# adityabalu/DiffNet

Hardware: NVIDIA B200
Metric: FEM loss+grad throughput (higher is better)
Workload: dtype f32

## Files before the change

diffnet_b200/csrc/dn_api.cu:

```cuda
#include <cstdarg>
#include <cstdio>
#include <cstdlib>
#include <cstring>

#include "dn_common.cuh"
#include "fem2d.cuh"
#include "fem2d_tma.cuh"
#include "fem3d.cuh"
#include "gp_eval.cuh"

namespace dn {
int debug_plan3t(const dn_geom* g, int nfields, int has_nu, int64_t* out);
cudaError_t launch_peer_put(float* dst_peer, const float* src, size_t n, int* remote_flag, int* local_counter,
                            unsigned int* ticket, cudaStream_t s);
cudaError_t launch_peer_wait(float* halo, const float* staged, size_t n, const int* flag, int* expect,
                             long long max_spins, int* status, cudaStream_t s);
cudaError_t launch_peer_loss_sum(const double* slots, int world, const int* step, long long max_spins, int* status,
                                 float* out, cudaStream_t s);
cudaError_t launch_peer_allreduce(const float* partial, float* out, double* slots, double* const* peer_slots,
                                  int rank, int world, int* counter, long long max_spins, int* status,
                                  cudaStream_t s);
}

namespace dn {
// ... 40 lines not shown
  }
  if (!g_dev[dev].ok) return fail(DN_EARCH, "device %d is not sm_100", dev);
  if (sms) *sms = g_dev[dev].sms;
  return DN_OK;
}

static int gauss_rule(int n, double* x, double* w) {
  switch (n) {
    case 2: x[0] = -0.5773502691896258; x[1] = 0.5773502691896258; w[0] = w[1] = 1.0; return 0;
    case 3: x[0] = -0.774596669; x[1] = 0.0; x[2] = 0.774596669;
            w[0] = 5.0 / 9.0; w[1] = 8.0 / 9.0; w[2] = 5.0 / 9.0; return 0;
    case 4: x[0] = -0.861136; x[1] = -0.339981; x[2] = 0.339981; x[3] = 0.861136;
            w[0] = 0.347855; w[1] = 0.652145; w[2] = 0.652145; w[3] = 0.347855; return 0;
  }
  return -1;
}

static Field to_field(const dn_field* f) {
  Field o{nullptr, 0, 0, 0};
  if (f && f->ptr) { o.p = f->ptr; o.sb = f->stride_b; o.sz = f->stride_z; o.sy = f->stride_y; }
  return o;
}

static bool aligned4(const Field& f, bool use_z) {
  if (!f.p) return true;
  return ((uintptr_t)f.p % 16 == 0) && (f.sb % 4 == 0) && (f.sy % 4 == 0) && (!use_z || f.sz % 4 == 0);
}

struct Common {
  Field u, nu, f, fgp, numask;
  Mask mk[DN_MAX_MASKS];
  int nmasks, MK;
  Consts k;
  Rule rule;
  bool vec4;
};

static int prepare(const dn_field* u, const dn_field* nu, const dn_field* f, const dn_field* fgp,
                   const dn_mask* masks, int nmasks, const dn_field* nu_zero_mask,
                   const dn_geom* g, double c_k, double c_f, double S, int nsd, Common* c, int flags = 0) {
  if (!g) return fail(DN_EINVAL, "geom is NULL");
  if (g->nsd != nsd) return fail(DN_EINVAL, "geom.nsd=%d but the %d-D entry point was called", g->nsd, nsd);
  if (g->batch < 1 || g->nx < 2 || g->ny < 2 || (nsd == 3 && g->nz < 2))
    return fail(DN_EINVAL, "need batch >= 1 and >= 2 nodes per direction (B=%d nx=%d ny=%d nz=%d)",
                g->batch, g->nx, g->ny, g->nz);
  if (!(g->hx > 0) || !(g->hy > 0) || (nsd == 3 && !(g->hz > 0)))
    return fail(DN_EINVAL, "element sizes must be positive");
  if (!u || !u->ptr) return fail(DN_EINVAL, "u is NULL");
  if (f && f->ptr && fgp && fgp->ptr) return fail(DN_EINVAL, "give f or fgp, not both");
  if ((flags & DN_F_LOAD_VECTOR) && !(f && f->ptr)) return fail(DN_EINVAL, "DN_F_LOAD_VECTOR needs the load vector in f");
  if (nmasks < 0 || nmasks > DN_MAX_MASKS)
    return fail(DN_EINVAL, "nmasks=%d (max %d)", nmasks, DN_MAX_MASKS);
  if (nmasks > 0 && !masks) return fail(DN_EINVAL, "masks is NULL");
  double gx[4], gw[4];
  if (gauss_rule(g->ngp_1d, gx, gw)) return fail(DN_EINVAL, "ngp_1d=%d (2..4)", g->ngp_1d);

  c->u = to_field(u); c->nu = to_field(nu); c->f = to_field(f); c->fgp = to_field(fgp);
  c->numask = to_field(nu_zero_mask);
  if (c->numask.p && !c->nu.p) return fail(DN_EINVAL, "nu_zero_mask needs nu");
  c->nmasks = nmasks;
  int nvf = 0;
  for (int i = 0; i < DN_MAX_MASKS; ++i) c->mk[i] = Mask{{nullptr, 0, 0, 0}, {nullptr, 0, 0, 0}, 0.f};
  for (int i = 0; i < nmasks; ++i) {
    if (!masks[i].mask.ptr) return fail(DN_EINVAL, "masks[%d].mask is NULL", i);
    c->mk[i].m = to_field(&masks[i].mask);
    c->mk[i].vf = to_field(&masks[i].value_field);
    c->mk[i].v = masks[i].value;
    nvf += c->mk[i].vf.p ? 1 : 0;
  }
  if (nvf > 0 && nmasks != 1)
    return fail(DN_EINVAL, "a Dirichlet value_field is supported only as the single mask");
  c->MK = nvf ? 4 : nmasks;

  double W1 = 0, m2 = 0;
  for (int i = 0; i < g->ngp_1d; ++i) { W1 += gw[i]; m2 += gw[i] * gx[i] * gx[i]; }
  const double t = m2 / W1;
  const double Wn = (nsd == 2) ? W1 * W1 : W1 * W1 * W1;
  const double nrm = (nsd == 2) ? 64.0 : 512.0;
  c->k.kx = (float)(S * c_k * Wn * (2.0 / g->hx) * (2.0 / g->hx) / nrm);
  c->k.ky = (float)(S * c_k * Wn * (2.0 / g->hy) * (2.0 / g->hy) / nrm);
  c->k.kz = (nsd == 3) ? (float)(S * c_k * Wn * (2.0 / g->hz) * (2.0 / g->hz) / nrm) : 0.f;
  c->k.kf = (float)(S * c_f * Wn / ((nsd == 2) ? 16.0 : 64.0));
  c->k.t = (float)t;
  c->k.kb = (float)(S * c_f);
  c->k.lv = (flags & DN_F_LOAD_VECTOR) ? 1 : 0;
  c->rule.n = g->ngp_1d;
  for (int i = 0; i < 4; ++i) {
    c->rule.x[i] = i < g->ngp_1d ? (float)gx[i] : 0.f;
    c->rule.w[i] = i < g->ngp_1d ? (float)gw[i] : 0.f;
  }
  c->rule.fscale = (float)(((nsd == 2) ? 4.0 : 8.0) / Wn);

  bool v4 = (g->nx % 4 == 0);
  const bool z = (nsd == 3);
  v4 = v4 && aligned4(c->u, z) && aligned4(c->nu, z) && aligned4(c->f, z) && aligned4(c->numask, z);
  for (int i = 0; i < nmasks; ++i) v4 = v4 && aligned4(c->mk[i].m, z) && aligned4(c->mk[i].vf, z);
  if (env_int("DN_FORCE_SCALAR", 0)) v4 = false;
  c->vec4 = v4;
  return DN_OK;
}

struct Plan2D { int V, R, nchunks, ntx, nitems, wpc, grid; };

static Plan2D plan2d(const dn_geom* g, bool vec4, int sms) {
  Plan2D pl;
  pl.V = vec4 ? 4 : 1;
  pl.ntx = (g->nx + 32 * pl.V - 1) / (32 * pl.V);
  const long long target = (long long)sms * env_int("DN_WARPS_PER_SM_2D", 16);
  long long per_row_items = (long long)g->batch * pl.ntx;
  long long want = (target + per_row_items - 1) / per_row_items;
  if (want < 1) want = 1;
  int R = (int)((g->ny + want - 1) / want);
  const int Rmin = env_int("DN_RMIN_2D", 8);
  if (R < Rmin) R = Rmin;
  if (R > g->ny) R = g->ny;
// ... 77 lines not shown
  if (!c.vec4 || c.fgp.p || ((uintptr_t)grad % 16 != 0)) return DN_OK;
  const int NU = c.nu.p ? 1 : 0, F = c.f.p ? (c.k.lv ? 2 : 1) : 0, NMK = c.numask.p ? 1 : 0;
  if (g->nx % 4 != 0 || g->nx / 4 > DN_T2_MAXT) return DN_OK;
  int MKx = c.MK;
  if (!mask_input) {
    if (c.MK == 0) MKx = 0;
    else if (c.MK >= 1 && c.MK <= 3 && !F && !NMK) MKx = c.MK + 4;
    else return DN_OK;
  }
  launch2t_fn fn = get_launch2t(MKx, NU, F, NMK);
  occ2t_fn occ = get_occ2t(MKx, NU, F, NMK);
  if (!fn || !occ) return DN_OK;
  P2T p;
  memset(&p, 0, sizeof(p));
  int nf = 0;
  p.fld[nf++] = c.u;
  if (NU) p.fld[nf++] = c.nu;
  if (F) p.fld[nf++] = c.f;
  if (NMK) p.fld[nf++] = c.numask;
  for (int i = 0; i < c.nmasks; ++i) { p.fld[nf++] = c.mk[i].m; p.mval[i] = c.mk[i].v; }
  if (c.MK == 4) p.fld[nf++] = c.mk[0].vf;
  for (int i = 0; i < nf; ++i)
    if (p.fld[i].sy != g->nx) return DN_OK;
  Plan2T pl = plan2t(g, nf, sms, occ);
  if (!pl.ok) { cudaGetLastError(); return DN_OK; }
  if (pl.grid > 0x7fffffffLL) return DN_OK;
  if (!workspace || wsb < ws_bytes_for_grid(pl.grid))
    return fail(DN_EWORKSPACE, "workspace too small: %zu < %zu", wsb, ws_bytes_for_grid(pl.grid));
  if ((uintptr_t)workspace % 16) return fail(DN_EWORKSPACE, "workspace must be 16-byte aligned");
  p.nf = nf;
  p.B = g->batch; p.nx = g->nx; p.ny = g->ny;
  p.R = pl.R; p.nchunks = pl.nchunks; p.S = pl.S;
  p.bal_q = pl.bal_q; p.bal_rem = pl.bal_rem;
  const float kx = c.k.kx, ky = c.k.ky, kf = c.k.kf, t = c.k.t;
  p.k2.kx = make_float2(kx, kx); p.k2.ky = make_float2(ky, ky); p.k2.t = make_float2(t, t);
  p.k2.kxt = make_float2(kx * t, kx * t); p.k2.kyt = make_float2(ky * t, ky * t);
  p.k2.nkf = make_float2(-kf, -kf); p.k2.nkft = make_float2(-kf * t, -kf * t);
  p.k2.nkftt = make_float2(-kf * t * t, -kf * t * t);
  p.k2.c0x_const = make_float2(4.f * kx, 4.f * kx); p.k2.c0y_const = make_float2(4.f * ky, 4.f * ky);
  p.k2.nkb = make_float2(-c.k.kb, -c.k.kb);
  p.grad = grad;
  p.red.counter = (unsigned int*)workspace;
  p.red.partials = (double*)((char*)workspace + 64);
  p.red.loss_out = loss_out; p.red.loss_f32 = loss_f32;
  p.mode = mode;
  *handled = true;
  return check_cuda(fn(p, dim3((unsigned)pl.grid), dim3(pl.threads), pl.smem, (cudaStream_t)stream),
                    "fem2d_tma launch");
}

static int run2d(const Common& c, const dn_geom* g, float* grad, float* grad_nu, int mode,
                 int mask_input, void* workspace, size_t wsb, double* loss_out, float* loss_f32,
                 void* stream, int sms) {
  if (!grad_nu) {
    bool handled = false;
    int rc = run2t(c, g, grad, mode, mask_input, workspace, wsb, loss_out, loss_f32, stream, sms, &handled);
    if (rc != DN_OK || handled) return rc;
  }
  if (c.k.lv)
    return fail(DN_ENOSTREAM, "DN_F_LOAD_VECTOR: the streaming 2-D kernel cannot take this launch (nx %% 4, nx <= %d, "
                "16-byte aligned dense rows, no grad_nu); pass f_gp instead", 4 * DN_T2_MAXT);
  bool vec4 = c.vec4 && ((uintptr_t)grad % 16 == 0) && ((uintptr_t)grad_nu % 16 == 0);
  Plan2D pl = plan2d(g, vec4, sms);
  if (!workspace || wsb < ws_bytes_for_grid(pl.grid))
    return fail(DN_EWORKSPACE, "workspace too small: %zu < %zu", wsb, ws_bytes_for_grid(pl.grid));
  if ((uintptr_t)workspace % 16) return fail(DN_EWORKSPACE, "workspace must be 16-byte aligned");
  P2D p;
  memset(&p, 0, sizeof(p));
  p.u = c.u; p.nu = c.nu; p.f = c.f; p.fgp = c.fgp; p.numask = c.numask;
  for (int i = 0; i < DN_MAX_MASKS; ++i) p.mk[i] = c.mk[i];
  p.B = g->batch; p.nx = g->nx; p.ny = g->ny;
// ... 396 lines not shown
```

diffnet_b200/csrc/fem2d_tma.cuh:

```cuda
#pragma once
#include <cstdlib>
#include <cstring>
#include <type_traits>

#include "dn_common.cuh"

namespace dn {

#define DN_T2_MAXF 8
#define DN_T2_MAXT 512

struct K2 {
  float2 kx, ky, kxt, kyt, t, nkf, nkft, nkftt, c0x_const, c0y_const;
  float2 nkb;
};

struct P2T {
  Field fld[DN_T2_MAXF];
  float mval[DN_MAX_MASKS];
  int nf;
  int B, nx, ny;
  int R, nchunks, S;
  int bal_q, bal_rem;
  K2 k2;
  float* grad;
  Reduce red;
  int mode;
};

__device__ __forceinline__ uint32_t smem_u32(const void* p) {
  return (uint32_t)__cvta_generic_to_shared(p);
}
__device__ __forceinline__ void mbar_init(uint64_t* bar, uint32_t count) {
  asm volatile("mbarrier.init.shared::cta.b64 [%0], %1;" ::"r"(smem_u32(bar)), "r"(count));
}
__device__ __forceinline__ void fence_mbar_init() {
  asm volatile("fence.mbarrier_init.release.cluster;" ::: "memory");
}
__device__ __forceinline__ void mbar_arrive_expect_tx(uint64_t* bar, uint32_t bytes) {
  asm volatile("mbarrier.arrive.expect_tx.shared::cta.b64 _, [%0], %1;" ::"r"(smem_u32(bar)),
               "r"(bytes)
               : "memory");
}
__device__ __forceinline__ void bulk_g2s(void* dst, const void* src, uint32_t bytes, uint64_t* bar) {
  asm volatile(
      "cp.async.bulk.shared::cluster.global.mbarrier::complete_tx::bytes [%0], [%1], %2, [%3];" ::"r"(
          smem_u32(dst)),
// ... 13 lines not shown
      "DN_DONE:\n"
      "}" ::"r"(smem_u32(bar)),
      "r"(parity)
      : "memory");
}

__device__ __forceinline__ void sts_if(bool pred, float* p, float v) {
  asm volatile("{\n.reg .pred P;\nsetp.ne.u32 P, %0, 0;\n@P st.shared.f32 [%1], %2;\n}" ::"r"((unsigned)pred), "r"(smem_u32(p)), "f"(v)
               : "memory");
}

__device__ __forceinline__ float2 f2(float a, float b) { return make_float2(a, b); }
__device__ __forceinline__ float2 f2(float a) { return make_float2(a, a); }
__device__ __forceinline__ float2 add2(float2 a, float2 b) { return __fadd2_rn(a, b); }
__device__ __forceinline__ float2 sub2(float2 a, float2 b) {
  return __fadd2_rn(a, make_float2(-b.x, -b.y));
}
__device__ __forceinline__ float2 mul2(float2 a, float2 b) { return __fmul2_rn(a, b); }
__device__ __forceinline__ float2 fma2(float2 a, float2 b, float2 c) { return __ffma2_rn(a, b, c); }

struct RowSD {
  float2 s01, s23, d01, d23;
};
__device__ __forceinline__ RowSD row_sd(const float (&v)[5]) {
  RowSD o;
  o.s01 = f2(v[0] + v[1], v[1] + v[2]);
  o.s23 = f2(v[2] + v[3], v[3] + v[4]);
  o.d01 = f2(v[1] - v[0], v[2] - v[1]);
  o.d23 = f2(v[3] - v[2], v[4] - v[3]);
  return o;
}


template <bool HAS_NU, bool HAS_F>
__device__ __forceinline__ float2 elem_pair(const K2& k, float2 st, float2 dt, float2 sb, float2 db,
                                            float2 nst, float2 ndt, float2 nsb, float2 ndb,
                                            float2 fst, float2 fdt, float2 fsb, float2 fdb,
                                            float2 vw, float2& ga, float2& gb, float2& gc,
                                            float2& gd) {
  const float2 Ae = sub2(sb, st), Ax = add2(dt, db), Axe = sub2(db, dt);
  float2 c0x, c0y, qx, qe, qxe;
  const float2 tAxe = mul2(k.t, Axe);
  if constexpr (HAS_NU) {
    const float2 C0 = add2(nst, nsb), Ce = sub2(nsb, nst), Cx = add2(ndt, ndb);
    c0x = mul2(k.kx, C0);
    c0y = mul2(k.ky, C0);
    const float2 c1x = mul2(k.kxt, Ce), c1y = mul2(k.kyt, Cx);
    qx = fma2(c0x, Ax, mul2(c1x, Axe));
    qe = fma2(c0y, Ae, mul2(c1y, Axe));
    qxe = fma2(add2(c0x, c0y), tAxe, fma2(c1x, Ax, mul2(c1y, Ae)));
  } else {
    c0x = mul2(k.c0x_const, vw);
    c0y = mul2(k.c0y_const, vw);
    qx = mul2(c0x, Ax);
    qe = mul2(c0y, Ae);
    qxe = mul2(add2(c0x, c0y), tAxe);
  }
  float2 E, g0, gx, ge, gxe;
  if constexpr (HAS_F) {
    const float2 A0 = add2(st, sb);
    const float2 nb0 = mul2(k.nkf, add2(fst, fsb));
    const float2 tx = fma2(k.nkft, add2(fdt, fdb), qx);
    const float2 te = fma2(k.nkft, sub2(fsb, fst), qe);
    const float2 txe = fma2(k.nkftt, sub2(fdb, fdt), qxe);
    E = fma2(A0, nb0, fma2(Ax, tx, fma2(Ae, te, mul2(Axe, txe))));
    g0 = nb0; gx = add2(qx, tx); ge = add2(qe, te); gxe = add2(qxe, txe);
    const float2 m0 = sub2(g0, ge), m1 = add2(g0, ge), n0 = sub2(gx, gxe), n1 = add2(gx, gxe);
    ga = sub2(m0, n0); gb = add2(m0, n0); gc = sub2(m1, n1); gd = add2(m1, n1);
  } else {
    E = fma2(Ax, qx, fma2(Ae, qe, mul2(Axe, qxe)));
    gx = add2(qx, qx); ge = add2(qe, qe); gxe = add2(qxe, qxe);
    const float2 n0 = sub2(gx, gxe), n1 = add2(gx, gxe);
    ga = sub2(f2(-ge.x, -ge.y), n0); gb = sub2(n0, ge); gc = sub2(ge, n1); gd = add2(ge, n1);
  }
  return E;
}

struct Row2T {
  RowSD u, n, f;
  float2 keep01, keep23;
  float2 lb01, lb23;
  float lE;
};
struct Acc2T {
  float2 a01, a23;
  float a4;
};

template <int NM, bool VF, bool HAS_NU, int FK, bool NUMASK, bool MI = true>
struct Fem2T {
  static constexpr bool HAS_F = (FK == 1), LV = (FK == 2);
  static constexpr int NF = 1 + (HAS_NU ? 1 : 0) + (FK ? 1 : 0) + (NUMASK ? 1 : 0) + NM + (VF ? 1 : 0);
  static constexpr int F_U = 0, F_NU = 1, F_F = F_NU + (HAS_NU ? 1 : 0), F_NM = F_F + (FK ? 1 : 0),
                       F_M = F_NM + (NUMASK ? 1 : 0), F_VF = F_M + NM;

  static __device__ __forceinline__ void load_row(const P2T& p, const float* __restrict__ sp, int fstride,
                                                  bool has_right, Row2T& o) {
    float v[NF][5];
#pragma unroll
    for (int f = 0; f < NF; ++f) {
      const float* q = sp + f * fstride;
      const float4 t = *reinterpret_cast<const float4*>(q);
      const float h = q[4];
      v[f][0] = t.x; v[f][1] = t.y; v[f][2] = t.z; v[f][3] = t.w; v[f][4] = has_right ? h : 0.f;
    }
    float ub[5], nb[5], fb[5], kp[4];
#pragma unroll
    for (int e = 0; e < 5; ++e) {
      float u = v[F_U][e];
      bool fx = false;
#pragma unroll
      for (int m = 0; m < NM; ++m) {
        const bool hit = v[F_M + m][e] > 0.5f;
        if constexpr (MI) u = hit ? (VF ? v[F_VF][e] : p.mval[m]) : u;
        fx = fx || hit;
      }
      ub[e] = u;
      if (e < 4) kp[e] = fx ? 0.f : 1.f;
      if constexpr (HAS_NU) {
        float n = v[F_NU][e];
        if constexpr (NUMASK) n = (v[F_NM][e] > 0.5f) ? 0.f : n;
        nb[e] = n;
      }
      if constexpr (HAS_F || LV) fb[e] = v[F_F][e];
    }
    o.keep01 = f2(kp[0], kp[1]);
    o.keep23 = f2(kp[2], kp[3]);
    if constexpr (LV) {
      o.lb01 = mul2(p.k2.nkb, f2(fb[0], fb[1]));
      o.lb23 = mul2(p.k2.nkb, f2(fb[2], fb[3]));
      const float2 le = fma2(o.lb01, f2(ub[0], ub[1]), mul2(o.lb23, f2(ub[2], ub[3])));
      o.lE = le.x + le.y;
    }
    o.u = row_sd(ub);
    if constexpr (HAS_NU) {
      o.n = row_sd(nb);
      if (!has_right) { o.n.s23.y = 0.f; o.n.d23.y = 0.f; }
    }
    if constexpr (HAS_F) {
      o.f = row_sd(fb);
      if (!has_right) { o.f.s23.y = 0.f; o.f.d23.y = 0.f; }
    }
  }

  static __device__ __forceinline__ float elem_row(const K2& k, const Row2T& top, const Row2T& bot,
                                                   float2 vw01, float2 vw23, Acc2T& At, Acc2T& Ab) {
    float2 ga, gb, gc, gd;
    const float2 E0 = elem_pair<HAS_NU, HAS_F>(k, top.u.s01, top.u.d01, bot.u.s01, bot.u.d01,
                                              top.n.s01, top.n.d01, bot.n.s01, bot.n.d01,
                                              top.f.s01, top.f.d01, bot.f.s01, bot.f.d01, vw01,
                                              ga, gb, gc, gd);
    At.a01 = add2(At.a01, ga);
    At.a01.y += gb.x; At.a23.x += gb.y;
    Ab.a01 = gc; Ab.a01.y += gd.x;
    const float carry = gd.y;
    const float2 E1 = elem_pair<HAS_NU, HAS_F>(k, top.u.s23, top.u.d23, bot.u.s23, bot.u.d23,
                                              top.n.s23, top.n.d23, bot.n.s23, bot.n.d23,
                                              top.f.s23, top.f.d23, bot.f.s23, bot.f.d23, vw23,
                                              ga, gb, gc, gd);
    At.a23 = add2(At.a23, ga);
    At.a23.y += gb.x; At.a4 += gb.y;
    Ab.a23 = gc; Ab.a23.x += carry; Ab.a23.y += gd.x;
    Ab.a4 = gd.y;
    const float2 Es = add2(E0, E1);
    return Es.x + Es.y;
  }
};

__device__ __forceinline__ unsigned int draw_start_ticket(const Reduce& r) { return atomicAdd(r.counter, 1u); }

__device__ __forceinline__ long long ld_relaxed_b64(const void* p) {
  long long v;
  asm volatile("ld.relaxed.gpu.global.b64 %0, [%1];" : "=l"(v) : "l"(p) : "memory");
  return v;
}

template <int NB = 40>
__device__ __forceinline__ void finish_loss_w0(const Reduce& r, double cta_value, unsigned int start_ticket) {
  if (threadIdx.x >= 32) return;
  const int lane = threadIdx.x;
  unsigned fin = 0u;
  if (lane == 0) {
    long long bits = __double_as_longlong(cta_value);
    if ((bits << 1) == 0) bits = (long long)0x8000000000000000ull;
    __stcg(reinterpret_cast<long long*>(r.partials + blockIdx.x), bits);
    fin = (start_ticket == gridDim.x - 1) ? 1u : 0u;
  }
  fin = __shfl_sync(0xffffffffu, fin, 0);
  if (!fin) return;
  const unsigned n = gridDim.x;
  double s = 0.0;
  for (unsigned base = 0; base < n; base += 32 * NB) {
// ... 42 lines not shown
  extern __shared__ __align__(128) unsigned char smem_raw[];
  __shared__ double s_red[TB / 32];
  __shared__ unsigned int s_ticket;

  const int tid = threadIdx.x, lane = tid & 31, warp = tid >> 5, nw = blockDim.x >> 5;
  const int nx = p.nx, S = p.S;
  const int stage_floats = NF * 2 * nx;
  float* ring = reinterpret_cast<float*>(smem_raw);
  uint64_t* full = reinterpret_cast<uint64_t*>(ring + (size_t)S * stage_floats + 4);
  float* seam = reinterpret_cast<float*>(full + S);

  int b, r_begin, r_end;
  if (p.bal_q > 0) {
    const int c = (int)blockIdx.x, hi = p.bal_rem * (p.bal_q + 1);
    int n, ch;
    if (c < hi) { n = p.bal_q + 1; b = c / n; ch = c - b * n; }
    else { n = p.bal_q; const int c2 = c - hi; b = c2 / n; ch = c2 - b * n; b += p.bal_rem; }
    r_begin = (int)((long long)ch * p.ny / n);
    r_end = (int)((long long)(ch + 1) * p.ny / n);
    if (!(p.ny & 1)) {
      if (ch > 0) r_begin |= 1;
      if (ch + 1 < n) r_end |= 1;
    }
  } else {
    b = blockIdx.x / p.nchunks;
    const int ch = blockIdx.x - b * p.nchunks;
    r_begin = ch * p.R;
    r_end = min(p.ny, r_begin + p.R);
  }
  const int j_first = max(r_begin - 1, 0), j_last = min(r_end, p.ny - 1);
  const int nrows = j_last - j_first + 1;
  const int nst = (nrows + 1) >> 1;

  int issued = 0, ist = 0;
  auto issue_stage = [&]() {
    if (tid == 0) {
      const int r0 = 2 * issued;
      const int nr = min(2, nrows - r0);
      const uint32_t row_bytes = (uint32_t)(nx * 4);
      uint64_t* bar = full + ist;
      float* dst = ring + ist * stage_floats;
      mbar_arrive_expect_tx(bar, (uint32_t)(NF * nr) * row_bytes);
#pragma unroll
      for (int f = 0; f < NF; ++f) {
        const float* src = p.fld[f].p + (long long)b * p.fld[f].sb + (long long)(j_first + r0) * nx;
        bulk_g2s(dst + f * 2 * nx, src, (uint32_t)nr * row_bytes, bar);
      }
    }
    ++issued;
    ist = (ist + 1 == S) ? 0 : ist + 1;
  };
  if (tid == 0) {
    for (int s = 0; s < S; ++s) mbar_init(full + s, 1);
    fence_mbar_init();
  }
  pdl_wait();
  {
    const int n0 = min(S, nst);
    for (int q = 0; q < n0; ++q) issue_stage();
  }
  if (tid == 0) s_ticket = draw_start_ticket(p.red);
  __syncthreads();

  const bool act = tid * 4 < nx;
  const int x0 = act ? tid * 4 : 0;
  const bool has_right = (x0 + 4) < nx;
  const float2 vw01 = f2(1.f, 1.f);
  const float2 vw23 = f2(1.f, has_right ? 1.f : 0.f);
  const K2& k = p.k2;
  const bool seam_in = (lane == 0) && (warp > 0);

  double acc = 0.0;
  int st = 0;
  uint32_t phase = 0;
  const float* sbase = ring + x0;
  float* gout = p.grad ? p.grad + ((long long)b * p.ny + j_first) * nx + x0 : nullptr;

  auto close_row = [&](const Acc2T& A, const Row2T& row, float4& G) {
    const float fromL = __shfl_up_sync(0xffffffffu, A.a4, 1);
    float2 g01 = A.a01, g23 = A.a23;
    if (lane > 0) g01.x += fromL;
    if constexpr (F::LV) { g01 = add2(g01, row.lb01); g23 = add2(g23, row.lb23); }
    g01 = mul2(g01, row.keep01);
    g23 = mul2(g23, row.keep23);
    G = make_float4(g01.x, g01.y, g23.x, g23.y);
  };
  const bool wr = act && (gout != nullptr), rs = act && (p.mode != 0), en = act && (p.mode == 0);
  float pend = 0.f;
  auto store_row = [&](float4 G, float keep0, float seam_v, const int jr, const bool inr, const float le) {
    G.x += seam_in ? seam_v * keep0 : 0.f;
    if (inr && wr) *reinterpret_cast<float4*>(gout + (long long)(jr - j_first) * nx) = G;
    const float sq = G.x * G.x + G.y * G.y + G.z * G.z + G.w * G.w;
    pend += (inr && rs) ? sq : 0.f;
    if constexpr (F::LV) pend += (inr && en) ? le : 0.f;
  };

  Row2T rowA, rowB;
  Acc2T accA, accB;
  accA.a01 = accA.a23 = f2(0.f); accA.a4 = 0.f;
  accB = accA;

  auto stage = [&](auto first_c, auto odd_c, const int q) {
    constexpr bool FIRST = decltype(first_c)::value, HAS_ODD = decltype(odd_c)::value;
    mbar_wait(full + st, phase);
    const float* sp = sbase + st * stage_floats;
    const int r0 = 2 * q;
    const int par = q & 1;
    float4 G0 = make_float4(0.f, 0.f, 0.f, 0.f), G1 = G0;
    float kp0 = 0.f, kp1 = 0.f, e = 0.f, le0 = 0.f, le1 = 0.f;

    F::load_row(p, sp, 2 * nx, has_right, rowA);
    if constexpr (!FIRST) {
      const float e0 = F::elem_row(k, rowB, rowA, vw01, vw23, accB, accA);
      e += (j_first + r0 - 1 >= r_begin) ? e0 : 0.f;
      sts_if(lane == 31, seam + (par * 2 + 0) * nw + warp, accB.a4);
      close_row(accB, rowB, G0);
      kp0 = rowB.keep01.x;
      if constexpr (F::LV) le0 = rowB.lE;
    }
    if constexpr (HAS_ODD) {
      F::load_row(p, sp + nx, 2 * nx, has_right, rowB);
      const float e1 = F::elem_row(k, rowA, rowB, vw01, vw23, accA, accB);
      e += (j_first + r0 >= r_begin) ? e1 : 0.f;
      sts_if(lane == 31, seam + (par * 2 + 1) * nw + warp, accA.a4);
      close_row(accA, rowA, G1);
      kp1 = rowA.keep01.x;
      if constexpr (F::LV) le1 = rowA.lE;
    }
    acc += (double)(((p.mode == 0 && act) ? e : 0.f) + pend);
    pend = 0.f;
    __syncthreads();
    if (issued < nst) issue_stage();
    ++st;
    if (st == S) { st = 0; phase ^= 1u; }
    const int wl = warp > 0 ? warp - 1 : 0;
    const float s0 = seam[(par * 2 + 0) * nw + wl];
    const float s1 = seam[(par * 2 + 1) * nw + wl];
    if constexpr (!FIRST) store_row(G0, kp0, s0, j_first + r0 - 1, true, le0);
    if constexpr (HAS_ODD) store_row(G1, kp1, s1, j_first + r0, FIRST ? (j_first >= r_begin) : true, le1);
  };
  const int nfull = nrows >> 1;
  stage(std::true_type{}, std::true_type{}, 0);
  for (int q = 1; q < nfull; ++q) stage(std::false_type{}, std::true_type{}, q);
  if (nrows & 1) stage(std::false_type{}, std::false_type{}, nfull);

  if (r_end == p.ny) {
    const bool lastB = (nrows & 1) == 0;
    const Acc2T& A = lastB ? accB : accA;
    const Row2T& row = lastB ? rowB : rowA;
    const int par = nst & 1;
    if (lane == 31) seam[(par * 2) * nw + warp] = A.a4;
    float4 G;
    close_row(A, row, G);
    __syncthreads();
    const float sv = seam_in ? seam[(par * 2) * nw + warp - 1] : 0.f;
    float le = 0.f;
    if constexpr (F::LV) le = row.lE;
    store_row(G, row.keep01.x, sv, p.ny - 1, true, le);
  }
  acc += (double)pend;

  pdl_trigger();
  acc = warp_sum(acc);
  if (lane == 0) s_red[warp] = acc;
  __syncthreads();
  double cta = 0.0;
  if (tid == 0)
    for (int w = 0; w < nw; ++w) cta += s_red[w];
  finish_loss_w0(p.red, cta, s_ticket);
}

typedef cudaError_t (*launch2t_fn)(const P2T&, dim3, dim3, size_t, cudaStream_t);
typedef int (*occ2t_fn)(int, size_t);
launch2t_fn get_launch2t(int MK, int NU, int F, int NUMASK);
occ2t_fn get_occ2t(int MK, int NU, int F, int NUMASK);

inline bool pdl_enabled() {
  static int v = -1;
  if (v < 0) { const char* e = getenv("DN_PDL"); v = (e && *e == '0') ? 0 : 1; }
  return v == 1;
}

constexpr int kMaxDynSmem = 226 * 1024;

template <int MK, bool HAS_NU, int FK, bool NUMASK>
struct Kern2T {
  static constexpr int NM = (MK == 4) ? 1 : (MK >= 5 ? MK - 4 : MK);
  static auto get() { return k_fem2d_tma<NM, (MK == 4), HAS_NU, FK, NUMASK, (MK < 5), DN_T2_MAXT, 1>; }
};

template <int MK, bool HAS_NU, int FK, bool NUMASK>
cudaError_t prep2t() {
// ... 37 lines not shown
```

Before: 195.7.

## Precompute nodal source load via separable stencil instead of per-element forcing terms

Removes the per-element forcing contribution from elem_pair and replaces it with a separable x/y stencil on the nodal f values. The x pass runs at row load (with a left-neighbour shared-memory read), and the y pass is carried across adjacent rows in row_source. Source energy is then added per node as 0.5*lb·u, and the forcing constants are precomputed on the host in double. The aim is fewer FMAs and registers in the hot element loop. The cost is extra boundary handling for the first and last rows, the left edge (xl) and the right edge (fxe), which risks boundary correctness.

```diff
diff --git a/diffnet_b200/csrc/dn_api.cu b/diffnet_b200/csrc/dn_api.cu
--- a/diffnet_b200/csrc/dn_api.cu
+++ b/diffnet_b200/csrc/dn_api.cu
@@ -96,6 +96,7 @@
   Mask mk[DN_MAX_MASKS];
   int nmasks, MK;
   Consts k;
+  double kf, t;
   Rule rule;
   bool vec4;
 };
@@ -144,7 +145,9 @@
   c->k.kx = (float)(S * c_k * Wn * (2.0 / g->hx) * (2.0 / g->hx) / nrm);
   c->k.ky = (float)(S * c_k * Wn * (2.0 / g->hy) * (2.0 / g->hy) / nrm);
   c->k.kz = (nsd == 3) ? (float)(S * c_k * Wn * (2.0 / g->hz) * (2.0 / g->hz) / nrm) : 0.f;
-  c->k.kf = (float)(S * c_f * Wn / ((nsd == 2) ? 16.0 : 64.0));
+  c->kf = S * c_f * Wn / ((nsd == 2) ? 16.0 : 64.0);
+  c->t = t;
+  c->k.kf = (float)c->kf;
   c->k.t = (float)t;
   c->k.kb = (float)(S * c_f);
   c->k.lv = (flags & DN_F_LOAD_VECTOR) ? 1 : 0;
@@ -288,11 +291,16 @@
   p.B = g->batch; p.nx = g->nx; p.ny = g->ny;
   p.R = pl.R; p.nchunks = pl.nchunks; p.S = pl.S;
   p.bal_q = pl.bal_q; p.bal_rem = pl.bal_rem;
-  const float kx = c.k.kx, ky = c.k.ky, kf = c.k.kf, t = c.k.t;
+  const float kx = c.k.kx, ky = c.k.ky, t = c.k.t;
+  auto pair = [](double v) { return make_float2((float)v, (float)v); };
   p.k2.kx = make_float2(kx, kx); p.k2.ky = make_float2(ky, ky); p.k2.t = make_float2(t, t);
   p.k2.kxt = make_float2(kx * t, kx * t); p.k2.kyt = make_float2(ky * t, ky * t);
-  p.k2.nkf = make_float2(-kf, -kf); p.k2.nkft = make_float2(-kf * t, -kf * t);
-  p.k2.nkftt = make_float2(-kf * t * t, -kf * t * t);
+  const double td = c.t, kfd = c.kf;
+  p.k2.fxa = pair(2.0 * (1.0 + td) / (1.0 - td));
+  p.k2.fxe = pair(-(1.0 + td) / (1.0 - td));
+  p.k2.fyn = pair(-kfd * (1.0 - td) * (1.0 - td));
+  p.k2.fyc = pair(-2.0 * kfd * (1.0 + td) * (1.0 - td));
+  p.k2.fye = pair(-kfd * (1.0 + td) * (1.0 - td));
   p.k2.c0x_const = make_float2(4.f * kx, 4.f * kx); p.k2.c0y_const = make_float2(4.f * ky, 4.f * ky);
   p.k2.nkb = make_float2(-c.k.kb, -c.k.kb);
   p.grad = grad;
diff --git a/diffnet_b200/csrc/fem2d_tma.cuh b/diffnet_b200/csrc/fem2d_tma.cuh
--- a/diffnet_b200/csrc/fem2d_tma.cuh
+++ b/diffnet_b200/csrc/fem2d_tma.cuh
@@ -11,8 +11,9 @@
 #define DN_T2_MAXT 512
 
 struct K2 {
-  float2 kx, ky, kxt, kyt, t, nkf, nkft, nkftt, c0x_const, c0y_const;
+  float2 kx, ky, kxt, kyt, t, c0x_const, c0y_const;
   float2 nkb;
+  float2 fxa, fxe, fyn, fyc, fye;
 };
 
 struct P2T {
@@ -92,10 +93,9 @@
 }
 
 
-template <bool HAS_NU, bool HAS_F>
+template <bool HAS_NU>
 __device__ __forceinline__ float2 elem_pair(const K2& k, float2 st, float2 dt, float2 sb, float2 db,
                                             float2 nst, float2 ndt, float2 nsb, float2 ndb,
-                                            float2 fst, float2 fdt, float2 fsb, float2 fdb,
                                             float2 vw, float2& ga, float2& gb, float2& gc,
                                             float2& gd) {
   const float2 Ae = sub2(sb, st), Ax = add2(dt, db), Axe = sub2(db, dt);
@@ -116,29 +116,17 @@
     qe = mul2(c0y, Ae);
     qxe = mul2(add2(c0x, c0y), tAxe);
   }
-  float2 E, g0, gx, ge, gxe;
-  if constexpr (HAS_F) {
-    const float2 A0 = add2(st, sb);
-    const float2 nb0 = mul2(k.nkf, add2(fst, fsb));
-    const float2 tx = fma2(k.nkft, add2(fdt, fdb), qx);
-    const float2 te = fma2(k.nkft, sub2(fsb, fst), qe);
-    const float2 txe = fma2(k.nkftt, sub2(fdb, fdt), qxe);
-    E = fma2(A0, nb0, fma2(Ax, tx, fma2(Ae, te, mul2(Axe, txe))));
-    g0 = nb0; gx = add2(qx, tx); ge = add2(qe, te); gxe = add2(qxe, txe);
-    const float2 m0 = sub2(g0, ge), m1 = add2(g0, ge), n0 = sub2(gx, gxe), n1 = add2(gx, gxe);
-    ga = sub2(m0, n0); gb = add2(m0, n0); gc = sub2(m1, n1); gd = add2(m1, n1);
-  } else {
-    E = fma2(Ax, qx, fma2(Ae, qe, mul2(Axe, qxe)));
-    gx = add2(qx, qx); ge = add2(qe, qe); gxe = add2(qxe, qxe);
-    const float2 n0 = sub2(gx, gxe), n1 = add2(gx, gxe);
-    ga = sub2(f2(-ge.x, -ge.y), n0); gb = sub2(n0, ge); gc = sub2(ge, n1); gd = add2(ge, n1);
-  }
+  const float2 E = fma2(Ax, qx, fma2(Ae, qe, mul2(Axe, qxe)));
+  const float2 gx = add2(qx, qx), ge = add2(qe, qe), gxe = add2(qxe, qxe);
+  const float2 n0 = sub2(gx, gxe), n1 = add2(gx, gxe);
+  ga = sub2(f2(-ge.x, -ge.y), n0); gb = sub2(n0, ge); gc = sub2(ge, n1); gd = add2(ge, n1);
   return E;
 }
 
 struct Row2T {
-  RowSD u, n, f;
+  RowSD u, n;
   float2 keep01, keep23;
+  float2 fx01, fx23;
   float2 lb01, lb23;
   float lE;
 };
@@ -155,7 +143,7 @@
                        F_M = F_NM + (NUMASK ? 1 : 0), F_VF = F_M + NM;
 
   static __device__ __forceinline__ void load_row(const P2T& p, const float* __restrict__ sp, int fstride,
-                                                  bool has_right, Row2T& o) {
+                                                  const float* __restrict__ spl, float xl, bool has_right, Row2T& o) {
     float v[NF][5];
 #pragma unroll
     for (int f = 0; f < NF; ++f) {
@@ -164,7 +152,7 @@
       const float h = q[4];
       v[f][0] = t.x; v[f][1] = t.y; v[f][2] = t.z; v[f][3] = t.w; v[f][4] = has_right ? h : 0.f;
     }
-    float ub[5], nb[5], fb[5], kp[4];
+    float ub[5], nb[5], kp[4];
 #pragma unroll
     for (int e = 0; e < 5; ++e) {
       float u = v[F_U][e];
@@ -182,13 +170,19 @@
         if constexpr (NUMASK) n = (v[F_NM][e] > 0.5f) ? 0.f : n;
         nb[e] = n;
       }
-      if constexpr (HAS_F || LV) fb[e] = v[F_F][e];
     }
     o.keep01 = f2(kp[0], kp[1]);
     o.keep23 = f2(kp[2], kp[3]);
+    if constexpr (HAS_F) {
+      const float* fv = v[F_F];
+      const float fl = fmaf(xl, fv[0], spl[F_F * fstride]);
+      const float fr = has_right ? fv[4] : p.k2.fxe.x * fv[3];
+      o.fx01 = fma2(p.k2.fxa, f2(fv[0], fv[1]), f2(fl + fv[1], fv[0] + fv[2]));
+      o.fx23 = fma2(p.k2.fxa, f2(fv[2], fv[3]), f2(fv[1] + fv[3], fv[2] + fr));
+    }
     if constexpr (LV) {
-      o.lb01 = mul2(p.k2.nkb, f2(fb[0], fb[1]));
-      o.lb23 = mul2(p.k2.nkb, f2(fb[2], fb[3]));
+      o.lb01 = mul2(p.k2.nkb, f2(v[F_F][0], v[F_F][1]));
+      o.lb23 = mul2(p.k2.nkb, f2(v[F_F][2], v[F_F][3]));
       const float2 le = fma2(o.lb01, f2(ub[0], ub[1]), mul2(o.lb23, f2(ub[2], ub[3])));
       o.lE = le.x + le.y;
     }
@@ -197,27 +191,39 @@
       o.n = row_sd(nb);
       if (!has_right) { o.n.s23.y = 0.f; o.n.d23.y = 0.f; }
     }
-    if constexpr (HAS_F) {
-      o.f = row_sd(fb);
-      if (!has_right) { o.f.s23.y = 0.f; o.f.d23.y = 0.f; }
-    }
+  }
+
+  template <bool FIRST>
+  static __device__ __forceinline__ void row_source(const K2& k, Row2T& above, Row2T& cur) {
+    if constexpr (FIRST) {
+      cur.lb01 = mul2(k.fye, cur.fx01);
+      cur.lb23 = mul2(k.fye, cur.fx23);
+    } else {
+      above.lb01 = fma2(k.fyn, cur.fx01, above.lb01);
+      above.lb23 = fma2(k.fyn, cur.fx23, above.lb23);
+      cur.lb01 = fma2(k.fyc, cur.fx01, mul2(k.fyn, above.fx01));
+      cur.lb23 = fma2(k.fyc, cur.fx23, mul2(k.fyn, above.fx23));
+    }
+  }
+
+  static __device__ __forceinline__ float src_energy(const Row2T& r, float e) {
+    const float2 le = fma2(r.lb01, sub2(r.u.s01, r.u.d01), mul2(r.lb23, sub2(r.u.s23, r.u.d23)));
+    return fmaf(0.5f, le.x + le.y, e);
   }
 
   static __device__ __forceinline__ float elem_row(const K2& k, const Row2T& top, const Row2T& bot,
                                                    float2 vw01, float2 vw23, Acc2T& At, Acc2T& Ab) {
     float2 ga, gb, gc, gd;
-    const float2 E0 = elem_pair<HAS_NU, HAS_F>(k, top.u.s01, top.u.d01, bot.u.s01, bot.u.d01,
-                                              top.n.s01, top.n.d01, bot.n.s01, bot.n.d01,
-                                              top.f.s01, top.f.d01, bot.f.s01, bot.f.d01, vw01,
-                                              ga, gb, gc, gd);
+    const float2 E0 = elem_pair<HAS_NU>(k, top.u.s01, top.u.d01, bot.u.s01, bot.u.d01,
+                                        top.n.s01, top.n.d01, bot.n.s01, bot.n.d01, vw01,
+                                        ga, gb, gc, gd);
     At.a01 = add2(At.a01, ga);
     At.a01.y += gb.x; At.a23.x += gb.y;
     Ab.a01 = gc; Ab.a01.y += gd.x;
     const float carry = gd.y;
-    const float2 E1 = elem_pair<HAS_NU, HAS_F>(k, top.u.s23, top.u.d23, bot.u.s23, bot.u.d23,
-                                              top.n.s23, top.n.d23, bot.n.s23, bot.n.d23,
-                                              top.f.s23, top.f.d23, bot.f.s23, bot.f.d23, vw23,
-                                              ga, gb, gc, gd);
+    const float2 E1 = elem_pair<HAS_NU>(k, top.u.s23, top.u.d23, bot.u.s23, bot.u.d23,
+                                        top.n.s23, top.n.d23, bot.n.s23, bot.n.d23, vw23,
+                                        ga, gb, gc, gd);
     At.a23 = add2(At.a23, ga);
     At.a23.y += gb.x; At.a4 += gb.y;
     Ab.a23 = gc; Ab.a23.x += carry; Ab.a23.y += gd.x;
@@ -368,13 +374,15 @@
   int st = 0;
   uint32_t phase = 0;
   const float* sbase = ring + x0;
+  const float* sbase_l = ring + (x0 > 0 ? x0 - 1 : 0);
+  const float xl = x0 > 0 ? 0.f : -1.f - 0.5f * p.k2.fxa.x;
   float* gout = p.grad ? p.grad + ((long long)b * p.ny + j_first) * nx + x0 : nullptr;
 
   auto close_row = [&](const Acc2T& A, const Row2T& row, float4& G) {
     const float fromL = __shfl_up_sync(0xffffffffu, A.a4, 1);
     float2 g01 = A.a01, g23 = A.a23;
     if (lane > 0) g01.x += fromL;
-    if constexpr (F::LV) { g01 = add2(g01, row.lb01); g23 = add2(g23, row.lb23); }
+    if constexpr (FK != 0) { g01 = add2(g01, row.lb01); g23 = add2(g23, row.lb23); }
     g01 = mul2(g01, row.keep01);
     g23 = mul2(g23, row.keep23);
     G = make_float4(g01.x, g01.y, g23.x, g23.y);
@@ -398,12 +406,14 @@
     constexpr bool FIRST = decltype(first_c)::value, HAS_ODD = decltype(odd_c)::value;
     mbar_wait(full + st, phase);
     const float* sp = sbase + st * stage_floats;
+    const float* spl = sbase_l + st * stage_floats;
     const int r0 = 2 * q;
     const int par = q & 1;
     float4 G0 = make_float4(0.f, 0.f, 0.f, 0.f), G1 = G0;
     float kp0 = 0.f, kp1 = 0.f, e = 0.f, le0 = 0.f, le1 = 0.f;
 
-    F::load_row(p, sp, 2 * nx, has_right, rowA);
+    F::load_row(p, sp, 2 * nx, spl, xl, has_right, rowA);
+    if constexpr (F::HAS_F) F::template row_source<FIRST>(k, rowB, rowA);
     if constexpr (!FIRST) {
       const float e0 = F::elem_row(k, rowB, rowA, vw01, vw23, accB, accA);
       e += (j_first + r0 - 1 >= r_begin) ? e0 : 0.f;
@@ -411,15 +421,18 @@
       close_row(accB, rowB, G0);
       kp0 = rowB.keep01.x;
       if constexpr (F::LV) le0 = rowB.lE;
+      if constexpr (F::HAS_F) e = F::src_energy(rowB, e);
     }
     if constexpr (HAS_ODD) {
-      F::load_row(p, sp + nx, 2 * nx, has_right, rowB);
+      F::load_row(p, sp + nx, 2 * nx, spl + nx, xl, has_right, rowB);
+      if constexpr (F::HAS_F) F::template row_source<false>(k, rowA, rowB);
       const float e1 = F::elem_row(k, rowA, rowB, vw01, vw23, accA, accB);
       e += (j_first + r0 >= r_begin) ? e1 : 0.f;
       sts_if(lane == 31, seam + (par * 2 + 1) * nw + warp, accA.a4);
       close_row(accA, rowA, G1);
       kp1 = rowA.keep01.x;
       if constexpr (F::LV) le1 = rowA.lE;
+      if constexpr (F::HAS_F) e = (FIRST && j_first < r_begin) ? e : F::src_energy(rowA, e);
     }
     acc += (double)(((p.mode == 0 && act) ? e : 0.f) + pend);
     pend = 0.f;
@@ -441,16 +454,19 @@
   if (r_end == p.ny) {
     const bool lastB = (nrows & 1) == 0;
     const Acc2T& A = lastB ? accB : accA;
-    const Row2T& row = lastB ? rowB : rowA;
+    Row2T row = lastB ? rowB : rowA;
+    if constexpr (F::HAS_F) {
+      row.lb01 = sub2(row.lb01, mul2(k.fye, row.fx01));
+      row.lb23 = sub2(row.lb23, mul2(k.fye, row.fx23));
+    }
     const int par = nst & 1;
     if (lane == 31) seam[(par * 2) * nw + warp] = A.a4;
     float4 G;
     close_row(A, row, G);
     __syncthreads();
     const float sv = seam_in ? seam[(par * 2) * nw + warp - 1] : 0.f;
-    float le = 0.f;
-    if constexpr (F::LV) le = row.lE;
-    store_row(G, row.keep01.x, sv, p.ny - 1, true, le);
+    store_row(G, row.keep01.x, sv, p.ny - 1, true, F::LV ? row.lE : 0.f);
+    if constexpr (F::HAS_F) pend += en ? F::src_energy(row, 0.f) : 0.f;
   }
   acc += (double)pend;
 
```

Result: faster. 201.4, median of 6 (+2.9%).

## Move forcing-term source assembly to separable nodal load vector in 2D TMA kernel

Applied to the files above, without the earlier changes.

Replaces the per-element forcing contribution inside elem_pair with a separable nodal load vector. Each row is filtered in x at load time, and that result is shared between adjacent rows in y through the carried xc01/xc23 terms. This takes the HAS_F arithmetic out of the element pair. The change also specialises the march loop on the residual/energy mode at compile time, which removes runtime mode branches. It also precomputes the per-field source pointers for TMA issue. Boundary handling now uses mirror coefficients and half-weight edge rows, which adds a risk of numerical or boundary mismatch.

```diff
diff --git a/diffnet_b200/csrc/dn_api.cu b/diffnet_b200/csrc/dn_api.cu
--- a/diffnet_b200/csrc/dn_api.cu
+++ b/diffnet_b200/csrc/dn_api.cu
@@ -291,8 +291,10 @@
   const float kx = c.k.kx, ky = c.k.ky, kf = c.k.kf, t = c.k.t;
   p.k2.kx = make_float2(kx, kx); p.k2.ky = make_float2(ky, ky); p.k2.t = make_float2(t, t);
   p.k2.kxt = make_float2(kx * t, kx * t); p.k2.kyt = make_float2(ky * t, ky * t);
-  p.k2.nkf = make_float2(-kf, -kf); p.k2.nkft = make_float2(-kf * t, -kf * t);
-  p.k2.nkftt = make_float2(-kf * t * t, -kf * t * t);
+  const float fc = 1.f - t, fw = 2.f * (1.f + t);
+  p.k2.nfc = make_float2(-kf * fc, -kf * fc); p.k2.nfw = make_float2(-kf * fw, -kf * fw);
+  p.k2.yc = make_float2(fc, fc); p.k2.yw = make_float2(fw, fw);
+  p.k2.fmir = make_float2(-(1.f + t) / fc, -(1.f + t) / fc);
   p.k2.c0x_const = make_float2(4.f * kx, 4.f * kx); p.k2.c0y_const = make_float2(4.f * ky, 4.f * ky);
   p.k2.nkb = make_float2(-c.k.kb, -c.k.kb);
   p.grad = grad;
diff --git a/diffnet_b200/csrc/fem2d_tma.cuh b/diffnet_b200/csrc/fem2d_tma.cuh
--- a/diffnet_b200/csrc/fem2d_tma.cuh
+++ b/diffnet_b200/csrc/fem2d_tma.cuh
@@ -11,7 +11,10 @@
 #define DN_T2_MAXT 512
 
 struct K2 {
-  float2 kx, ky, kxt, kyt, t, nkf, nkft, nkftt, c0x_const, c0y_const;
+  float2 kx, ky, kxt, kyt, t, c0x_const, c0y_const;
+  float2 nfc, nfw;
+  float2 fmir;
+  float2 yc, yw;
   float2 nkb;
 };
 
@@ -92,10 +95,9 @@
 }
 
 
-template <bool HAS_NU, bool HAS_F>
+template <bool HAS_NU>
 __device__ __forceinline__ float2 elem_pair(const K2& k, float2 st, float2 dt, float2 sb, float2 db,
                                             float2 nst, float2 ndt, float2 nsb, float2 ndb,
-                                            float2 fst, float2 fdt, float2 fsb, float2 fdb,
                                             float2 vw, float2& ga, float2& gb, float2& gc,
                                             float2& gd) {
   const float2 Ae = sub2(sb, st), Ax = add2(dt, db), Axe = sub2(db, dt);
@@ -116,31 +118,19 @@
     qe = mul2(c0y, Ae);
     qxe = mul2(add2(c0x, c0y), tAxe);
   }
-  float2 E, g0, gx, ge, gxe;
-  if constexpr (HAS_F) {
-    const float2 A0 = add2(st, sb);
-    const float2 nb0 = mul2(k.nkf, add2(fst, fsb));
-    const float2 tx = fma2(k.nkft, add2(fdt, fdb), qx);
-    const float2 te = fma2(k.nkft, sub2(fsb, fst), qe);
-    const float2 txe = fma2(k.nkftt, sub2(fdb, fdt), qxe);
-    E = fma2(A0, nb0, fma2(Ax, tx, fma2(Ae, te, mul2(Axe, txe))));
-    g0 = nb0; gx = add2(qx, tx); ge = add2(qe, te); gxe = add2(qxe, txe);
-    const float2 m0 = sub2(g0, ge), m1 = add2(g0, ge), n0 = sub2(gx, gxe), n1 = add2(gx, gxe);
-    ga = sub2(m0, n0); gb = add2(m0, n0); gc = sub2(m1, n1); gd = add2(m1, n1);
-  } else {
-    E = fma2(Ax, qx, fma2(Ae, qe, mul2(Axe, qxe)));
-    gx = add2(qx, qx); ge = add2(qe, qe); gxe = add2(qxe, qxe);
-    const float2 n0 = sub2(gx, gxe), n1 = add2(gx, gxe);
-    ga = sub2(f2(-ge.x, -ge.y), n0); gb = sub2(n0, ge); gc = sub2(ge, n1); gd = add2(ge, n1);
-  }
+  const float2 E = fma2(Ax, qx, fma2(Ae, qe, mul2(Axe, qxe)));
+  const float2 gx = add2(qx, qx), ge = add2(qe, qe), gxe = add2(qxe, qxe);
+  const float2 n0 = sub2(gx, gxe), n1 = add2(gx, gxe);
+  ga = sub2(f2(-ge.x, -ge.y), n0); gb = sub2(n0, ge); gc = sub2(ge, n1); gd = add2(ge, n1);
   return E;
 }
 
 struct Row2T {
-  RowSD u, n, f;
+  RowSD u, n;
   float2 keep01, keep23;
   float2 lb01, lb23;
   float lE;
+  float2 fx01, fx23;
 };
 struct Acc2T {
   float2 a01, a23;
@@ -150,12 +140,13 @@
 template <int NM, bool VF, bool HAS_NU, int FK, bool NUMASK, bool MI = true>
 struct Fem2T {
   static constexpr bool HAS_F = (FK == 1), LV = (FK == 2);
+  static constexpr bool NODAL = HAS_F || LV;
   static constexpr int NF = 1 + (HAS_NU ? 1 : 0) + (FK ? 1 : 0) + (NUMASK ? 1 : 0) + NM + (VF ? 1 : 0);
   static constexpr int F_U = 0, F_NU = 1, F_F = F_NU + (HAS_NU ? 1 : 0), F_NM = F_F + (FK ? 1 : 0),
                        F_M = F_NM + (NUMASK ? 1 : 0), F_VF = F_M + NM;
 
   static __device__ __forceinline__ void load_row(const P2T& p, const float* __restrict__ sp, int fstride,
-                                                  bool has_right, Row2T& o) {
+                                                  bool has_left, bool has_right, Row2T& o) {
     float v[NF][5];
 #pragma unroll
     for (int f = 0; f < NF; ++f) {
@@ -164,6 +155,8 @@
       const float h = q[4];
       v[f][0] = t.x; v[f][1] = t.y; v[f][2] = t.z; v[f][3] = t.w; v[f][4] = has_right ? h : 0.f;
     }
+    float fl = 0.f;
+    if constexpr (HAS_F) fl = sp[F_F * fstride - 1];
     float ub[5], nb[5], fb[5], kp[4];
 #pragma unroll
     for (int e = 0; e < 5; ++e) {
@@ -192,32 +185,42 @@
       const float2 le = fma2(o.lb01, f2(ub[0], ub[1]), mul2(o.lb23, f2(ub[2], ub[3])));
       o.lE = le.x + le.y;
     }
+    if constexpr (HAS_F) {
+      fl = has_left ? fl : p.k2.fmir.x * fb[0];
+      const float fr = has_right ? fb[4] : p.k2.fmir.x * fb[3];
+      o.fx01 = fma2(p.k2.nfc, f2(fl + fb[1], fb[0] + fb[2]), mul2(p.k2.nfw, f2(fb[0], fb[1])));
+      o.fx23 = fma2(p.k2.nfc, f2(fb[1] + fb[3], fb[2] + fr), mul2(p.k2.nfw, f2(fb[2], fb[3])));
+    }
     o.u = row_sd(ub);
     if constexpr (HAS_NU) {
       o.n = row_sd(nb);
       if (!has_right) { o.n.s23.y = 0.f; o.n.d23.y = 0.f; }
     }
-    if constexpr (HAS_F) {
-      o.f = row_sd(fb);
-      if (!has_right) { o.f.s23.y = 0.f; o.f.d23.y = 0.f; }
-    }
+  }
+
+  static __device__ __forceinline__ void src_share(const K2& k, float2 xa01, float2 xa23, float2 xb01,
+                                                   float2 xb23, float2 wy, Row2T& row) {
+    row.lb01 = fma2(k.yc, add2(xa01, xb01), mul2(wy, row.fx01));
+    row.lb23 = fma2(k.yc, add2(xa23, xb23), mul2(wy, row.fx23));
+    const float2 ls = f2(row.lb01.x + row.lb01.y, row.lb23.x + row.lb23.y);
+    const float2 ld = f2(row.lb01.y - row.lb01.x, row.lb23.y - row.lb23.x);
+    const float2 le = fma2(f2(row.u.s01.x, row.u.s23.x), ls, mul2(f2(row.u.d01.x, row.u.d23.x), ld));
+    row.lE = 0.5f * (le.x + le.y);
   }
 
   static __device__ __forceinline__ float elem_row(const K2& k, const Row2T& top, const Row2T& bot,
                                                    float2 vw01, float2 vw23, Acc2T& At, Acc2T& Ab) {
     float2 ga, gb, gc, gd;
-    const float2 E0 = elem_pair<HAS_NU, HAS_F>(k, top.u.s01, top.u.d01, bot.u.s01, bot.u.d01,
-                                              top.n.s01, top.n.d01, bot.n.s01, bot.n.d01,
-                                              top.f.s01, top.f.d01, bot.f.s01, bot.f.d01, vw01,
-                                              ga, gb, gc, gd);
+    const float2 E0 = elem_pair<HAS_NU>(k, top.u.s01, top.u.d01, bot.u.s01, bot.u.d01,
+                                        top.n.s01, top.n.d01, bot.n.s01, bot.n.d01, vw01,
+                                        ga, gb, gc, gd);
     At.a01 = add2(At.a01, ga);
     At.a01.y += gb.x; At.a23.x += gb.y;
     Ab.a01 = gc; Ab.a01.y += gd.x;
     const float carry = gd.y;
-    const float2 E1 = elem_pair<HAS_NU, HAS_F>(k, top.u.s23, top.u.d23, bot.u.s23, bot.u.d23,
-                                              top.n.s23, top.n.d23, bot.n.s23, bot.n.d23,
-                                              top.f.s23, top.f.d23, bot.f.s23, bot.f.d23, vw23,
-                                              ga, gb, gc, gd);
+    const float2 E1 = elem_pair<HAS_NU>(k, top.u.s23, top.u.d23, bot.u.s23, bot.u.d23,
+                                        top.n.s23, top.n.d23, bot.n.s23, bot.n.d23, vw23,
+                                        ga, gb, gc, gd);
     At.a23 = add2(At.a23, ga);
     At.a23.y += gb.x; At.a4 += gb.y;
     Ab.a23 = gc; Ab.a23.x += carry; Ab.a23.y += gd.x;
@@ -326,21 +329,22 @@
   const int nrows = j_last - j_first + 1;
   const int nst = (nrows + 1) >> 1;
 
+  const uint32_t row_bytes = (uint32_t)(nx * 4);
+  const float* src[NF];
+#pragma unroll
+  for (int f = 0; f < NF; ++f) src[f] = p.fld[f].p + (long long)b * p.fld[f].sb + (long long)j_first * nx;
   int issued = 0, ist = 0;
   auto issue_stage = [&]() {
     if (tid == 0) {
-      const int r0 = 2 * issued;
-      const int nr = min(2, nrows - r0);
-      const uint32_t row_bytes = (uint32_t)(nx * 4);
+      const uint32_t nr_bytes = (issued + 1 < nst || !(nrows & 1)) ? 2 * row_bytes : row_bytes;
       uint64_t* bar = full + ist;
       float* dst = ring + ist * stage_floats;
-      mbar_arrive_expect_tx(bar, (uint32_t)(NF * nr) * row_bytes);
-#pragma unroll
-      for (int f = 0; f < NF; ++f) {
-        const float* src = p.fld[f].p + (long long)b * p.fld[f].sb + (long long)(j_first + r0) * nx;
-        bulk_g2s(dst + f * 2 * nx, src, (uint32_t)nr * row_bytes, bar);
-      }
-    }
+      mbar_arrive_expect_tx(bar, (uint32_t)NF * nr_bytes);
+#pragma unroll
+      for (int f = 0; f < NF; ++f) bulk_g2s(dst + f * 2 * nx, src[f], nr_bytes, bar);
+    }
+#pragma unroll
+    for (int f = 0; f < NF; ++f) src[f] += 2 * nx;
     ++issued;
     ist = (ist + 1 == S) ? 0 : ist + 1;
   };
@@ -358,10 +362,12 @@
 
   const bool act = tid * 4 < nx;
   const int x0 = act ? tid * 4 : 0;
-  const bool has_right = (x0 + 4) < nx;
+  const bool has_right = (x0 + 4) < nx, has_left = x0 > 0;
   const float2 vw01 = f2(1.f, 1.f);
   const float2 vw23 = f2(1.f, has_right ? 1.f : 0.f);
   const K2& k = p.k2;
+  const float2 wy_edge = mul2(f2(0.5f), k.yw);
+  float2 xc01 = f2(0.f), xc23 = f2(0.f);
   const bool seam_in = (lane == 0) && (warp > 0);
 
   double acc = 0.0;
@@ -374,19 +380,22 @@
     const float fromL = __shfl_up_sync(0xffffffffu, A.a4, 1);
     float2 g01 = A.a01, g23 = A.a23;
     if (lane > 0) g01.x += fromL;
-    if constexpr (F::LV) { g01 = add2(g01, row.lb01); g23 = add2(g23, row.lb23); }
+    if constexpr (F::NODAL) { g01 = add2(g01, row.lb01); g23 = add2(g23, row.lb23); }
     g01 = mul2(g01, row.keep01);
     g23 = mul2(g23, row.keep23);
     G = make_float4(g01.x, g01.y, g23.x, g23.y);
   };
-  const bool wr = act && (gout != nullptr), rs = act && (p.mode != 0), en = act && (p.mode == 0);
+  const bool wr = act && (gout != nullptr);
   float pend = 0.f;
-  auto store_row = [&](float4 G, float keep0, float seam_v, const int jr, const bool inr, const float le) {
+  auto store_row = [&](auto res_c, float4 G, float keep0, float seam_v, const int jr, const bool inr, const float le) {
     G.x += seam_in ? seam_v * keep0 : 0.f;
     if (inr && wr) *reinterpret_cast<float4*>(gout + (long long)(jr - j_first) * nx) = G;
-    const float sq = G.x * G.x + G.y * G.y + G.z * G.z + G.w * G.w;
-    pend += (inr && rs) ? sq : 0.f;
-    if constexpr (F::LV) pend += (inr && en) ? le : 0.f;
+    if constexpr (decltype(res_c)::value) {
+      const float sq = G.x * G.x + G.y * G.y + G.z * G.z + G.w * G.w;
+      pend += (inr && act) ? sq : 0.f;
+    } else if constexpr (F::NODAL) {
+      pend += (inr && act) ? le : 0.f;
+    }
   };
 
   Row2T rowA, rowB;
@@ -394,8 +403,8 @@
   accA.a01 = accA.a23 = f2(0.f); accA.a4 = 0.f;
   accB = accA;
 
-  auto stage = [&](auto first_c, auto odd_c, const int q) {
-    constexpr bool FIRST = decltype(first_c)::value, HAS_ODD = decltype(odd_c)::value;
+  auto stage = [&](auto first_c, auto odd_c, auto res_c, const int q) {
+    constexpr bool FIRST = decltype(first_c)::value, HAS_ODD = decltype(odd_c)::value, RES = decltype(res_c)::value;
     mbar_wait(full + st, phase);
     const float* sp = sbase + st * stage_floats;
     const int r0 = 2 * q;
@@ -403,25 +412,33 @@
     float4 G0 = make_float4(0.f, 0.f, 0.f, 0.f), G1 = G0;
     float kp0 = 0.f, kp1 = 0.f, e = 0.f, le0 = 0.f, le1 = 0.f;
 
-    F::load_row(p, sp, 2 * nx, has_right, rowA);
+    F::load_row(p, sp, 2 * nx, has_left, has_right, rowA);
     if constexpr (!FIRST) {
       const float e0 = F::elem_row(k, rowB, rowA, vw01, vw23, accB, accA);
       e += (j_first + r0 - 1 >= r_begin) ? e0 : 0.f;
       sts_if(lane == 31, seam + (par * 2 + 0) * nw + warp, accB.a4);
+      if constexpr (F::HAS_F) {
+        F::src_share(k, xc01, xc23, rowA.fx01, rowA.fx23, k.yw, rowB);
+        xc01 = rowB.fx01; xc23 = rowB.fx23;
+      }
       close_row(accB, rowB, G0);
       kp0 = rowB.keep01.x;
-      if constexpr (F::LV) le0 = rowB.lE;
+      if constexpr (F::NODAL) le0 = rowB.lE;
     }
     if constexpr (HAS_ODD) {
-      F::load_row(p, sp + nx, 2 * nx, has_right, rowB);
+      F::load_row(p, sp + nx, 2 * nx, has_left, has_right, rowB);
       const float e1 = F::elem_row(k, rowA, rowB, vw01, vw23, accA, accB);
       e += (j_first + r0 >= r_begin) ? e1 : 0.f;
       sts_if(lane == 31, seam + (par * 2 + 1) * nw + warp, accA.a4);
+      if constexpr (F::HAS_F) {
+        F::src_share(k, xc01, xc23, rowB.fx01, rowB.fx23, FIRST ? wy_edge : k.yw, rowA);
+        xc01 = rowA.fx01; xc23 = rowA.fx23;
+      }
       close_row(accA, rowA, G1);
       kp1 = rowA.keep01.x;
-      if constexpr (F::LV) le1 = rowA.lE;
-    }
-    acc += (double)(((p.mode == 0 && act) ? e : 0.f) + pend);
+      if constexpr (F::NODAL) le1 = rowA.lE;
+    }
+    acc += (double)(((!RES && act) ? e : 0.f) + pend);
     pend = 0.f;
     __syncthreads();
     if (issued < nst) issue_stage();
@@ -430,28 +447,33 @@
     const int wl = warp > 0 ? warp - 1 : 0;
     const float s0 = seam[(par * 2 + 0) * nw + wl];
     const float s1 = seam[(par * 2 + 1) * nw + wl];
-    if constexpr (!FIRST) store_row(G0, kp0, s0, j_first + r0 - 1, true, le0);
-    if constexpr (HAS_ODD) store_row(G1, kp1, s1, j_first + r0, FIRST ? (j_first >= r_begin) : true, le1);
+    if constexpr (!FIRST) store_row(res_c, G0, kp0, s0, j_first + r0 - 1, true, le0);
+    if constexpr (HAS_ODD) store_row(res_c, G1, kp1, s1, j_first + r0, FIRST ? (j_first >= r_begin) : true, le1);
   };
-  const int nfull = nrows >> 1;
-  stage(std::true_type{}, std::true_type{}, 0);
-  for (int q = 1; q < nfull; ++q) stage(std::false_type{}, std::true_type{}, q);
-  if (nrows & 1) stage(std::false_type{}, std::false_type{}, nfull);
-
-  if (r_end == p.ny) {
-    const bool lastB = (nrows & 1) == 0;
-    const Acc2T& A = lastB ? accB : accA;
-    const Row2T& row = lastB ? rowB : rowA;
-    const int par = nst & 1;
-    if (lane == 31) seam[(par * 2) * nw + warp] = A.a4;
-    float4 G;
-    close_row(A, row, G);
-    __syncthreads();
-    const float sv = seam_in ? seam[(par * 2) * nw + warp - 1] : 0.f;
-    float le = 0.f;
-    if constexpr (F::LV) le = row.lE;
-    store_row(G, row.keep01.x, sv, p.ny - 1, true, le);
-  }
+  auto march = [&](auto res_c) {
+    const int nfull = nrows >> 1;
+    stage(std::true_type{}, std::true_type{}, res_c, 0);
+    for (int q = 1; q < nfull; ++q) stage(std::false_type{}, std::true_type{}, res_c, q);
+    if (nrows & 1) stage(std::false_type{}, std::false_type{}, res_c, nfull);
+
+    if (r_end == p.ny) {
+      const bool lastB = (nrows & 1) == 0;
+      const Acc2T& A = lastB ? accB : accA;
+      Row2T row = lastB ? rowB : rowA;
+      const int par = nst & 1;
+      if (lane == 31) seam[(par * 2) * nw + warp] = A.a4;
+      if constexpr (F::HAS_F) F::src_share(k, xc01, xc23, f2(0.f), f2(0.f), wy_edge, row);
+      float4 G;
+      close_row(A, row, G);
+      __syncthreads();
+      const float sv = seam_in ? seam[(par * 2) * nw + warp - 1] : 0.f;
+      float le = 0.f;
+      if constexpr (F::NODAL) le = row.lE;
+      store_row(res_c, G, row.keep01.x, sv, p.ny - 1, true, le);
+    }
+  };
+  if (p.mode != 0) march(std::true_type{});
+  else march(std::false_type{});
   acc += (double)pend;
 
   pdl_trigger();
```

Result: faster. 195.9 before, 204.6 after (median of 6 runs) (+4.4%).
